# ai-dynamo/dynamo

Hardware: AMD Instinct MI355X
Metric: output tok/s (node), Llama-3-70B serving, ISL8192/OSL1024, conc 16/GPU (higher is better)
Workload: dtype bf16; 1 GPU; model=llama-3-70b, global_batch=16, seq_len=8192, osl=1024, parallelism=agg1, kv_cache_dtype=auto

## Files before the change

dynamo_amd/csrc/activation.hip:

```cpp
#include "common.h"
#include <torch/extension.h>
#include <ATen/hip/HIPContext.h>

namespace {

constexpr int kBlock = 256;

__global__ void silu_mul_kernel(short* __restrict__ out,
                                const short* __restrict__ gu,
                                int64_t T, int64_t I) {
  const int64_t nvec = T * (I / 8);
  for (int64_t v = (int64_t)blockIdx.x * kBlock + threadIdx.x; v < nvec;
       v += (int64_t)gridDim.x * kBlock) {
    const int64_t t = v / (I / 8);
    const int64_t i0 = (v % (I / 8)) * 8;
    short8 g = *reinterpret_cast<const short8*>(gu + t * 2 * I + i0);
    short8 u = *reinterpret_cast<const short8*>(gu + t * 2 * I + I + i0);
    short8 o;
#pragma unroll
    for (int i = 0; i < 8; i++) {
      float gf = bf16_to_f32(g[i]);
      float uf = bf16_to_f32(u[i]);
      float s = gf / (1.f + __expf(-gf));
      o[i] = f32_to_bf16(s * uf);
    }
    *reinterpret_cast<short8*>(out + t * I + i0) = o;
  }
}

__global__ void gelu_kernel(short* __restrict__ out, const short* __restrict__ in,
                            int64_t n) {
  const int64_t nvec = n / 8;
  for (int64_t v = (int64_t)blockIdx.x * kBlock + threadIdx.x; v < nvec;
       v += (int64_t)gridDim.x * kBlock) {
    short8 x = *reinterpret_cast<const short8*>(in + v * 8);
    short8 o;
#pragma unroll
    for (int i = 0; i < 8; i++) {
      float xf = bf16_to_f32(x[i]);
      float c = 0.7978845608028654f * (xf + 0.044715f * xf * xf * xf);
      o[i] = f32_to_bf16(0.5f * xf * (1.f + tanhf(c)));
    }
    *reinterpret_cast<short8*>(out + v * 8) = o;
  }
}

}

void silu_mul(torch::Tensor out, torch::Tensor gate_up) {
  TORCH_CHECK(out.is_cuda() && out.dtype() == torch::kBFloat16);
  TORCH_CHECK(gate_up.is_contiguous() && out.is_contiguous());
  const int64_t I = out.size(-1);
  const int64_t T = out.numel() / I;
  TORCH_CHECK(gate_up.size(-1) == 2 * I && I % 8 == 0);
  if (T == 0) return;
  const int64_t nvec = T * (I / 8);
  const int grid = (int)std::min<int64_t>((nvec + kBlock - 1) / kBlock, 2048);
  auto stream = at::cuda::getCurrentHIPStream();
// ... 17 lines not shown
```

dynamo_amd/csrc/bindings.cpp:

```cpp
#include <torch/extension.h>
#include <pybind11/pybind11.h>

namespace py = pybind11;

void rmsnorm(torch::Tensor out, torch::Tensor input, torch::Tensor weight,
             double eps, bool allow_fast);
void fused_add_rmsnorm(torch::Tensor input, torch::Tensor residual,
                       torch::Tensor weight, double eps, bool allow_fast);
void rope_append_qkv(torch::Tensor q_out, torch::Tensor kcache,
                     torch::Tensor vcache, torch::Tensor qkv,
                     c10::optional<torch::Tensor> bias,
                     torch::Tensor positions, torch::Tensor slot_mapping,
                     torch::Tensor cos_sin_cache, bool v_transposed,
                     bool allow_fast);
void rope_inplace(torch::Tensor q, torch::Tensor k, torch::Tensor positions,
                  torch::Tensor cos_sin_cache, int64_t num_q_heads,
                  int64_t num_k_heads, int64_t head_dim);
void silu_mul(torch::Tensor out, torch::Tensor gate_up);
void gelu(torch::Tensor out, torch::Tensor input);
void kv_cache_append(torch::Tensor kcache, torch::Tensor vcache, torch::Tensor k,
                     torch::Tensor v, torch::Tensor slot_mapping,
                     bool v_transposed);
void gather_pages(torch::Tensor staging, torch::Tensor cache, torch::Tensor page_ids);
void scatter_pages(torch::Tensor staging, torch::Tensor cache, torch::Tensor page_ids);
void copy_pages(torch::Tensor dst_cache, torch::Tensor src_cache, torch::Tensor pairs);
int64_t paged_decode_num_chunks(int64_t max_ctx);
int64_t decode_chunk_tokens_py(int64_t max_ctx);
void paged_attention_decode(torch::Tensor out, torch::Tensor q, torch::Tensor kcache,
                            torch::Tensor vcache, torch::Tensor page_table,
                            torch::Tensor ctx_lens, torch::Tensor partial,
                            torch::Tensor ml, double scale,
                            int64_t chunk_tokens, bool v_transposed,
                            int64_t nt_policy);
void attention_prefill_paged(torch::Tensor out, torch::Tensor q,
                             torch::Tensor kcache, torch::Tensor vcache,
                             torch::Tensor page_table, torch::Tensor tile_seq,
                             torch::Tensor tile_q0, torch::Tensor seq_q_start,
                             torch::Tensor seq_q_len, torch::Tensor seq_ctx_len,
                             double scale, bool v_transposed);
void greedy_sample(torch::Tensor out, torch::Tensor logits, bool allow_fast);
void topkp_sample(torch::Tensor out, torch::Tensor logits,
                  torch::Tensor inv_temp, torch::Tensor top_k,
                  torch::Tensor top_p, int64_t seed,
                  c10::optional<torch::Tensor> row_seeds);
void gumbel_sample(torch::Tensor out, torch::Tensor logits, torch::Tensor inv_temp,
                   int64_t seed, c10::optional<torch::Tensor> row_seeds,
                   bool allow_fast);
void penalty_fold(torch::Tensor counts, torch::Tensor slot,
                  torch::Tensor token, torch::Tensor is_prompt);
void logits_process(torch::Tensor logits, c10::optional<torch::Tensor> counts,
                    torch::Tensor slot, torch::Tensor params,
                    c10::optional<torch::Tensor> bias_off,
                    c10::optional<torch::Tensor> bias_ids,
                    c10::optional<torch::Tensor> bias_vals, bool allow_fast);
void skinny_gemm(torch::Tensor y, torch::Tensor x, torch::Tensor w,
                 int64_t wpb, int64_t u, int64_t nt, bool nontemporal,
                 bool coalesced);
std::map<std::string, std::vector<std::tuple<int, int, int>>>
skinny_gemm_configs();
void fp8_skinny_gemm(torch::Tensor y, torch::Tensor x, torch::Tensor wq,
                     torch::Tensor scale, int64_t wpb, int64_t u, int64_t nt,
                     bool nontemporal);
void fp8_dequant(torch::Tensor out, torch::Tensor wq, torch::Tensor scale);
void mxfp4_skinny_gemm(torch::Tensor y, torch::Tensor x, torch::Tensor q,
                       torch::Tensor scale, int64_t wpb, int64_t u,
                       int64_t nt, bool nontemporal);
int64_t mxfp4_gemm_max_m();
void mxfp4_dequant(torch::Tensor out, torch::Tensor q, torch::Tensor scale);
void lora_shrink(torch::Tensor t, torch::Tensor x, torch::Tensor A_bank,
                 torch::Tensor slots, torch::Tensor ranks);
void lora_expand_add(torch::Tensor y, torch::Tensor t, torch::Tensor B_bank,
                     torch::Tensor slots, torch::Tensor ranks,
                     torch::Tensor scales);
void moe_grouped_gemm(torch::Tensor y, torch::Tensor x, torch::Tensor w,
                      torch::Tensor tiles);
void moe_grouped_gemm_seg(torch::Tensor y, torch::Tensor x, torch::Tensor w,
                          torch::Tensor seg_start, int64_t max_tokens);
void topk_gating(torch::Tensor topw, torch::Tensor topi, torch::Tensor logits);
torch::Tensor ipc_alloc(int64_t nbytes, int64_t device);
py::bytes ipc_export(torch::Tensor t);
torch::Tensor ipc_open(py::bytes handle_bytes, int64_t nbytes, int64_t device);
void enable_peer_access(int64_t device, int64_t peer);
torch::Tensor mfma_probe(torch::Tensor A, torch::Tensor B);
torch::Tensor tr16_probe();
torch::Tensor vstage_probe();
torch::Tensor pv_probe(int64_t hot);

PYBIND11_MODULE(TORCH_EXTENSION_NAME, m) {
  m.doc() = "dynamo_amd native MI355X (gfx950) kernels";
  m.def("rmsnorm", &rmsnorm, py::arg("out"), py::arg("input"),
        py::arg("weight"), py::arg("eps"), py::arg("allow_fast") = true);
  m.def("fused_add_rmsnorm", &fused_add_rmsnorm, py::arg("input"),
        py::arg("residual"), py::arg("weight"), py::arg("eps"),
        py::arg("allow_fast") = true);
  m.def("rope_inplace", &rope_inplace);
  m.def("rope_append_qkv", &rope_append_qkv,
        py::arg("q_out"), py::arg("kcache"), py::arg("vcache"),
        py::arg("qkv"), py::arg("bias"), py::arg("positions"),
        py::arg("slot_mapping"), py::arg("cos_sin"),
// ... 4 lines not shown
        py::arg("vcache"), py::arg("k"), py::arg("v"),
        py::arg("slot_mapping"), py::arg("v_transposed") = false);
  m.def("gather_pages", &gather_pages);
  m.def("scatter_pages", &scatter_pages);
  m.def("copy_pages", &copy_pages);
  m.def("paged_decode_num_chunks", &paged_decode_num_chunks);
  m.def("decode_chunk_tokens", &decode_chunk_tokens_py);
  m.def("paged_attention_decode", &paged_attention_decode,
        py::arg("out"), py::arg("q"), py::arg("kcache"), py::arg("vcache"),
        py::arg("page_table"), py::arg("ctx_lens"), py::arg("partial"),
        py::arg("ml"), py::arg("scale"), py::arg("chunk_tokens"),
        py::arg("v_transposed") = false, py::arg("nt_policy") = -1);
  m.def("attention_prefill_paged", &attention_prefill_paged,
        py::arg("out"), py::arg("q"), py::arg("kcache"), py::arg("vcache"),
        py::arg("page_table"), py::arg("tile_seq"), py::arg("tile_q0"),
        py::arg("seq_q_start"), py::arg("seq_q_len"), py::arg("seq_ctx_len"),
        py::arg("scale"), py::arg("v_transposed") = false);
  m.def("greedy_sample", &greedy_sample, py::arg("out"), py::arg("logits"),
        py::arg("allow_fast") = true);
  m.def("gumbel_sample", &gumbel_sample, py::arg("out"), py::arg("logits"),
        py::arg("inv_temp"), py::arg("seed"),
        py::arg("row_seeds") = py::none(), py::arg("allow_fast") = true);
  m.def("topkp_sample", &topkp_sample, py::arg("out"), py::arg("logits"),
        py::arg("inv_temp"), py::arg("top_k"), py::arg("top_p"),
        py::arg("seed"), py::arg("row_seeds") = py::none());
  m.def("penalty_fold", &penalty_fold, py::arg("counts"), py::arg("slot"),
        py::arg("token"), py::arg("is_prompt"));
  m.def("logits_process", &logits_process, py::arg("logits"),
        py::arg("counts"), py::arg("slot"), py::arg("params"),
        py::arg("bias_off") = py::none(), py::arg("bias_ids") = py::none(),
        py::arg("bias_vals") = py::none(), py::arg("allow_fast") = true);
  m.def("skinny_gemm", &skinny_gemm, py::arg("y"), py::arg("x"), py::arg("w"),
        py::arg("wpb") = 4, py::arg("u") = 4, py::arg("nt") = 2,
        py::arg("nontemporal") = false, py::arg("coalesced") = false);
  m.def("fp8_skinny_gemm", &fp8_skinny_gemm, py::arg("y"), py::arg("x"),
        py::arg("wq"), py::arg("scale"), py::arg("wpb") = 1, py::arg("u") = 1,
        py::arg("nt") = 2, py::arg("nontemporal") = true);
  m.def("fp8_dequant", &fp8_dequant, py::arg("out"), py::arg("wq"),
        py::arg("scale"));
  m.def("mxfp4_skinny_gemm", &mxfp4_skinny_gemm, py::arg("y"), py::arg("x"),
        py::arg("q"), py::arg("scale"), py::arg("wpb") = 1, py::arg("u") = 1,
        py::arg("nt") = 2, py::arg("nontemporal") = true);
  m.def("mxfp4_gemm_max_m", &mxfp4_gemm_max_m);
  m.def("mxfp4_dequant", &mxfp4_dequant, py::arg("out"), py::arg("q"),
        py::arg("scale"));
  m.def("skinny_gemm_configs", &skinny_gemm_configs);
  m.def("lora_shrink", &lora_shrink, py::arg("t"), py::arg("x"),
        py::arg("A_bank"), py::arg("slots"), py::arg("ranks"));
  m.def("lora_expand_add", &lora_expand_add, py::arg("y"), py::arg("t"),
        py::arg("B_bank"), py::arg("slots"), py::arg("ranks"),
        py::arg("scales"));
  m.def("moe_grouped_gemm", &moe_grouped_gemm);
  m.def("moe_grouped_gemm_seg", &moe_grouped_gemm_seg);
  m.def("topk_gating", &topk_gating);
  m.def("ipc_alloc", &ipc_alloc);
  m.def("ipc_export", &ipc_export);
  m.def("ipc_open", &ipc_open);
  m.def("enable_peer_access", &enable_peer_access);
  m.def("mfma_probe", &mfma_probe);
  m.def("tr16_probe", &tr16_probe);
  m.def("vstage_probe", &vstage_probe);
  m.def("pv_probe", &pv_probe);
}
```

dynamo_amd/csrc/common.h:

```cpp
#pragma once

#include <hip/hip_runtime.h>
#include <hip/hip_bf16.h>
#include <hip/hip_fp16.h>
#include <stdint.h>

#define WAVE_SIZE 64

#define DEVINL __device__ __forceinline__

typedef __attribute__((ext_vector_type(8))) short short8;
typedef __attribute__((ext_vector_type(4))) short short4v;
typedef __attribute__((ext_vector_type(4))) float float4v;
typedef __attribute__((ext_vector_type(2))) float float2v;

typedef __attribute__((ext_vector_type(8))) short bf16x8;
typedef __attribute__((ext_vector_type(4))) float f32x4;
typedef __attribute__((ext_vector_type(16))) float f32x16;

DEVINL float bf16_to_f32(short u) {
  union { float f; uint32_t i; } v;
  v.i = ((uint32_t)(uint16_t)u) << 16;
  return v.f;
}

DEVINL short f32_to_bf16(float f) {
  union { float f; uint32_t i; } v;
  v.f = f;
  uint32_t lsb = (v.i >> 16) & 1;
  uint32_t rounded = v.i + 0x7fff + lsb;
  return (short)(rounded >> 16);
}

DEVINL float wave_reduce_sum(float x) {
#pragma unroll
  for (int off = 32; off > 0; off >>= 1) x += __shfl_xor(x, off, WAVE_SIZE);
  return x;
}

DEVINL float wave_reduce_max(float x) {
#pragma unroll
  for (int off = 32; off > 0; off >>= 1) x = fmaxf(x, __shfl_xor(x, off, WAVE_SIZE));
  return x;
}

template <int WIDTH>
DEVINL float group_reduce_sum(float x) {
#pragma unroll
  for (int off = WIDTH / 2; off > 0; off >>= 1) x += __shfl_xor(x, off, WAVE_SIZE);
  return x;
}

DEVINL float block_reduce_sum(float x, float* lds_scratch) {
  const int lane = threadIdx.x & (WAVE_SIZE - 1);
  const int wid = threadIdx.x / WAVE_SIZE;
  const int nwaves = blockDim.x / WAVE_SIZE;
  x = wave_reduce_sum(x);
  if (lane == 0) lds_scratch[wid] = x;
  __syncthreads();
  float total = 0.f;
  if (threadIdx.x < (unsigned)nwaves) total = lds_scratch[threadIdx.x];
  if (wid == 0) {
#pragma unroll
    for (int off = 8; off > 0; off >>= 1) total += __shfl_xor(total, off, WAVE_SIZE);
// ... 75 lines not shown
```

dynamo_amd/csrc/skinny_gemm.hip:

```cpp
#include "skinny_gemm_impl.h"
#include <torch/extension.h>
#include <ATen/hip/HIPContext.h>

namespace {

struct GemmArgs {
  const short* x;
  const void* w;
  const void* scale;
  short* y;
  int M, N, K;
  int64_t wpb, u, nt;
  bool nontemporal;
};

GemmArgs check_args(const char* name, int64_t max_m, int64_t min_k,
                    int64_t k_per_step, const torch::Tensor& y,
                    const torch::Tensor& x, const torch::Tensor& w,
                    const torch::Tensor* scale, int64_t wpb, int64_t u,
                    int64_t nt, bool nontemporal, int64_t w_pack = 1,
                    bool block_scaled = false) {
  TORCH_CHECK(x.is_cuda() && w.is_cuda() && y.is_cuda() &&
                  (!scale || scale->is_cuda()),
              name, ": tensors must be on the GPU");
  TORCH_CHECK(x.dtype() == torch::kBFloat16 && y.dtype() == torch::kBFloat16,
              name, ": x and y must be bf16");
  TORCH_CHECK(x.dim() == 2 && w.dim() == 2 && y.dim() == 2 &&
                  (!scale || scale->dim() == (block_scaled ? 2 : 1)),
              name, ": x [M,K], w [N,K], scale [N], y [M,N]");
  TORCH_CHECK(x.is_contiguous() && w.is_contiguous() && y.is_contiguous() &&
                  (!scale || scale->is_contiguous()),
              name, ": tensors must be contiguous");
  const int64_t M = x.size(0), K = x.size(1), N = w.size(0);
  TORCH_CHECK(w.size(1) * w_pack == K && y.size(0) == M && y.size(1) == N &&
                  (!scale || scale->size(0) == N) &&
                  (!block_scaled || scale->size(1) * 32 == K),
              name, ": shape mismatch");
  TORCH_CHECK(M >= 1 && M <= max_m, name, ": needs 1 <= M <= ", max_m,
              ", got ", M);
  TORCH_CHECK(N >= 16 && N % 16 == 0, name, ": needs N % 16 == 0, got ", N);
  TORCH_CHECK(N < (1 << 27), name, ": N too large");
  TORCH_CHECK(wpb > 0 && u > 0 && nt > 0, name, ": bad configuration");
  const int64_t kstep = wpb * k_per_step * u;
  TORCH_CHECK(K >= min_k && K < (1 << 30) && K % kstep == 0, name,
              ": needs K >= ", min_k, " and K % ", kstep, " == 0, got ", K);
  TORCH_CHECK((uintptr_t)x.data_ptr() % 16 == 0 &&
                  (uintptr_t)w.data_ptr() % 16 == 0,
              name, ": x and w must be 16 B aligned");
  TORCH_CHECK(!block_scaled || (uintptr_t)scale->data_ptr() % 8 == 0, name,
              ": scale must be 8 B aligned");
  return {(const short*)x.data_ptr(), w.data_ptr(),
          scale ? scale->data_ptr() : nullptr,
          (short*)y.data_ptr(), (int)M, (int)N, (int)K, wpb, u, nt,
          nontemporal};
}

template <class F, int WPB, int U, int NT, int MT>
void launch(const GemmArgs& a) {
  if constexpr (MT > 1) {
    if (a.M <= (MT - 1) * 16) return launch<F, WPB, U, NT, MT - 1>(a);
  }
  const int grid = (a.N + NT * 16 - 1) / (NT * 16);
  auto stream = at::cuda::getCurrentHIPStream();
  auto w = (const typename F::welem*)a.w;
  auto scale = (const typename F::scale_t*)a.scale;
  if (a.nontemporal)
    skinny::skinny_gemm_kernel<F, WPB, U, NT, MT, 1>
        <<<grid, WPB * 64, 0, stream>>>(a.x, w, scale, a.y, a.M, a.N, a.K);
  else
    skinny::skinny_gemm_kernel<F, WPB, U, NT, MT, 0>
        <<<grid, WPB * 64, 0, stream>>>(a.x, w, scale, a.y, a.M, a.N, a.K);
}

typedef std::vector<std::tuple<int, int, int>> ConfigList;

#define GEMM_CASE(WPB, U, NT)                                                \
  if (a.wpb == WPB && a.u == U && a.nt == NT)                                \
    return launch<Format, WPB, U, NT, kMaxMt>(a);
#define GEMM_ENTRY(WPB, U, NT) {WPB, U, NT},
#define GEMM_DISPATCH(NAME, F, MAX_MT, TABLE)                                \
  void NAME(const char* name, const GemmArgs& a) {                           \
    using Format = F;                                                        \
    constexpr int kMaxMt = MAX_MT;                                           \
    TABLE(GEMM_CASE)                                                         \
    TORCH_CHECK(false, name, ": no kernel for (WPB, U, NT) = (", a.wpb,      \
                ", ", a.u, ", ", a.nt, ")");                                 \
  }                                                                          \
  ConfigList NAME##_configs() { return {TABLE(GEMM_ENTRY)}; }
GEMM_DISPATCH(launch_plain, skinny::Bf16Plain, 1, SKINNY_GEMM_CONFIGS)
GEMM_DISPATCH(launch_coal, skinny::Bf16Coal, 1, SKINNY_GEMM_COAL_CONFIGS)
GEMM_DISPATCH(launch_fp8, skinny::Fp8Coal, 4, FP8_GEMM_CONFIGS)
GEMM_DISPATCH(launch_mxfp4, skinny::Mxfp4Coal, MXFP4_GEMM_MAX_MT,
              MXFP4_GEMM_CONFIGS)
#undef GEMM_DISPATCH
#undef GEMM_ENTRY
#undef GEMM_CASE

}

void skinny_gemm(torch::Tensor y, torch::Tensor x, torch::Tensor w,
                 int64_t wpb, int64_t u, int64_t nt, bool nontemporal,
                 bool coalesced) {
  const char* name = "skinny_gemm";
  TORCH_CHECK(w.dtype() == torch::kBFloat16, name, ": w must be bf16");
  const GemmArgs a = check_args(
      name, 16, 2048,
      coalesced ? skinny::Bf16Coal::KSTEP : skinny::Bf16Plain::KSTEP, y, x, w,
      nullptr, wpb, u, nt, nontemporal);
  if (coalesced) launch_coal(name, a);
  else launch_plain(name, a);
  HIP_CHECK_KERNEL();
}

void fp8_skinny_gemm(torch::Tensor y, torch::Tensor x, torch::Tensor wq,
                     torch::Tensor scale, int64_t wpb, int64_t u, int64_t nt,
                     bool nontemporal) {
  const char* name = "fp8_skinny_gemm";
  TORCH_CHECK(wq.dtype() == at::kFloat8_e4m3fn, name,
              ": wq must be float8_e4m3fn");
  TORCH_CHECK(scale.dtype() == torch::kFloat32, name, ": scale must be fp32");
  launch_fp8(name, check_args(name, 64, 128, skinny::Fp8Coal::KSTEP, y, x, wq,
                              &scale, wpb, u, nt, nontemporal));
  HIP_CHECK_KERNEL();
}

void mxfp4_skinny_gemm(torch::Tensor y, torch::Tensor x, torch::Tensor q,
                       torch::Tensor scale, int64_t wpb, int64_t u,
                       int64_t nt, bool nontemporal) {
  const char* name = "mxfp4_skinny_gemm";
  TORCH_CHECK(q.dtype() == torch::kUInt8 && scale.dtype() == torch::kUInt8,
              name, ": q and scale must be uint8");
  launch_mxfp4(name, check_args(name, 16 * MXFP4_GEMM_MAX_MT, 256,
                                skinny::Mxfp4Coal::KSTEP, y, x, q, &scale,
                                wpb, u, nt, nontemporal,
                                skinny::Mxfp4Coal::WPACK, true));
  HIP_CHECK_KERNEL();
}

std::map<std::string, ConfigList> skinny_gemm_configs() {
  return {{"bf16_plain", launch_plain_configs()},
          {"bf16_coalesced", launch_coal_configs()},
          {"fp8", launch_fp8_configs()},
          {"mxfp4", launch_mxfp4_configs()}};
}

int64_t mxfp4_gemm_max_m() { return 16 * MXFP4_GEMM_MAX_MT; }

void fp8_dequant(torch::Tensor out, torch::Tensor wq, torch::Tensor scale) {
  TORCH_CHECK(out.is_cuda() && wq.is_cuda() && scale.is_cuda(),
              "fp8_dequant: tensors must be on the GPU");
  TORCH_CHECK(out.dtype() == torch::kBFloat16 &&
                  wq.dtype() == at::kFloat8_e4m3fn &&
                  scale.dtype() == torch::kFloat32,
              "fp8_dequant: out bf16, wq float8_e4m3fn, scale fp32");
  TORCH_CHECK(out.dim() == 2 && wq.dim() == 2 && scale.dim() == 1,
              "fp8_dequant: out [N,K], wq [N,K], scale [N]");
  TORCH_CHECK(out.is_contiguous() && wq.is_contiguous() &&
                  scale.is_contiguous(),
              "fp8_dequant: tensors must be contiguous");
  const int64_t N = wq.size(0), K = wq.size(1);
  TORCH_CHECK(out.size(0) == N && out.size(1) == K && scale.size(0) == N,
              "fp8_dequant: shape mismatch");
  TORCH_CHECK(N >= 1 && K >= 16 && K % 16 == 0,
              "fp8_dequant: needs K % 16 == 0, got ", K);
  TORCH_CHECK((uintptr_t)out.data_ptr() % 16 == 0 &&
                  (uintptr_t)wq.data_ptr() % 16 == 0,
              "fp8_dequant: out and wq must be 16 B aligned");
  const int64_t threads = N * (K / 16);
  const int64_t blocks = (threads + 255) / 256;
  TORCH_CHECK(blocks < (1ll << 31), "fp8_dequant: matrix too large");
  auto stream = at::cuda::getCurrentHIPStream();
  skinny::fp8_dequant_kernel<<<(unsigned)blocks, 256, 0, stream>>>(
      (short*)out.data_ptr(), (const unsigned char*)wq.data_ptr(),
      (const float*)scale.data_ptr(), (long long)N, (long long)K);
  HIP_CHECK_KERNEL();
}
// ... 31 lines not shown
```

dynamo_amd/csrc/skinny_gemm_impl.h:

```cpp
#pragma once

#include "common.h"

namespace skinny {

typedef __attribute__((ext_vector_type(4))) int int4v;

template <int NTL>
DEVINL int4v ldw(const void* p) {
  if constexpr (NTL)
    return __builtin_nontemporal_load(reinterpret_cast<const int4v*>(p));
  else
    return *reinterpret_cast<const int4v*>(p);
}

#if !defined(__HIP_DEVICE_COMPILE__)
DEVINL bf16x8 e4m3x8_to_bf16x8(int, int) { return bf16x8{}; }
#else
DEVINL bf16x8 e4m3x8_to_bf16x8(int w0, int w1) {
  const float2v f[4] = {__builtin_amdgcn_cvt_pk_f32_fp8(w0, false),
                        __builtin_amdgcn_cvt_pk_f32_fp8(w0, true),
                        __builtin_amdgcn_cvt_pk_f32_fp8(w1, false),
                        __builtin_amdgcn_cvt_pk_f32_fp8(w1, true)};
  unsigned int out[4];
#pragma unroll
  for (int i = 0; i < 4; i++) {
    const float lo = f[i].x, hi = f[i].y;
    out[i] = __builtin_amdgcn_perm(__float_as_uint(hi), __float_as_uint(lo),
                                   0x07060302u);
  }
  return *reinterpret_cast<bf16x8*>(out);
}
#endif

typedef __attribute__((ext_vector_type(2))) __bf16 bf16x2;
// ... 66 lines not shown
  typedef CoalSel Sel;
  static constexpr int KSTEP = 128, LOADS = 2, FRAGS = 4, WPACK = 1;
  static constexpr bool SCALED = true, BLOCK_SCALED = false;
  static DEVINL int w_row(int lane, int h) { return coal_w_row(lane, h); }
  static DEVINL int w_k(int lane) { return (lane & 7) * 16; }
  static DEVINL int x_k(int lane) { return (lane >> 4) * 16; }
  static constexpr int x_step(int s) { return 64 * (s >> 1) + 8 * (s & 1); }
  static DEVINL Sel sel(int lane) { return coal_sel(lane); }
  static DEVINL bf16x8 b_frag(int s, const int4v (&r)[2], Sel l, Aux) {
    return e4m3x8_to_bf16x8(coal_take(l, s >> 1, r, 2 * (s & 1)),
                            coal_take(l, s >> 1, r, 2 * (s & 1) + 1));
  }
};

typedef __attribute__((ext_vector_type(2))) unsigned int uint2v;
struct Mxfp4Coal {
  typedef unsigned char welem;
  typedef unsigned char scale_t;
  typedef uint2v Aux;
  struct Sel { CoalSel c; int shift; };
  static constexpr int KSTEP = 256, LOADS = 2, FRAGS = 8, WPACK = 2;
  static constexpr bool SCALED = false, BLOCK_SCALED = true;
  static DEVINL int w_row(int lane, int h) { return coal_w_row(lane, h); }
  static DEVINL int w_k(int lane) { return (lane & 7) * 16; }
  static DEVINL int x_k(int lane) { return (lane >> 4) * 32; }
  static constexpr int x_step(int s) { return 128 * (s >> 2) + 8 * (s & 3); }
  static DEVINL Sel sel(int lane) { return {coal_sel(lane), (lane >> 4) * 8}; }
  static DEVINL bf16x8 b_frag(int s, const int4v (&r)[2], Sel l, Aux a) {
    return e2m1x8_to_bf16x8(coal_take(l.c, s >> 2, r, s & 3),
                            (a[s >> 2] >> l.shift) & 0xffu);
  }
};

template <class F, int WPB, int U, int NT, int MT, int NTL>
__global__ __launch_bounds__(WPB * 64) void skinny_gemm_kernel(
    const short* __restrict__ x,
    const typename F::welem* __restrict__ w,
    const typename F::scale_t* __restrict__ scale,
    short* __restrict__ y,
    int M, int N, int K) {
  const int lane = threadIdx.x & 63;
  const int wid = threadIdx.x >> 6;
  const int lr = lane & 15;
  const int lg = lane >> 4;
  const int n0 = (blockIdx.x * NT) * 16;
  if (n0 >= N) return;

  const int kw = K / WPB;
  const int k0 = wid * kw;
  const int steps = kw / F::KSTEP;

  const short* xp[MT];
#pragma unroll
  for (int m = 0; m < MT; m++) {
    const int row = m * 16 + lr;
    xp[m] = x + (size_t)(row < M ? row : 0) * K + k0 + F::x_k(lane);
  }
  const typename F::welem* wp[NT][F::LOADS];
#pragma unroll
  for (int t = 0; t < NT; t++)
#pragma unroll
    for (int h = 0; h < F::LOADS; h++) {
      const int col = n0 + t * 16 + F::w_row(lane, h);
      wp[t][h] = w + (size_t)(col < N ? col : N - 1) * (K / F::WPACK) +
                 k0 / F::WPACK + F::w_k(lane);
    }
  const typename F::scale_t* sp[NT];
  if constexpr (F::BLOCK_SCALED) {
#pragma unroll
    for (int t = 0; t < NT; t++) {
      const int col = n0 + t * 16 + lr;
      sp[t] = scale + ((size_t)(col < N ? col : N - 1) * K + k0) / 32;
    }
  }

  const typename F::Sel sel = F::sel(lane);

  f32x4 acc[NT][MT];
#pragma unroll
  for (int t = 0; t < NT; t++)
#pragma unroll
    for (int m = 0; m < MT; m++) acc[t][m] = f32x4{0.f, 0.f, 0.f, 0.f};

  bf16x8 abuf[U][MT][F::FRAGS];
  int4v rbuf[NT][U][F::LOADS];
  typename F::Aux auxbuf[NT][U];
  auto load_x = [&](bf16x8 (&a)[MT][F::FRAGS], int d) {
#pragma unroll
    for (int m = 0; m < MT; m++)
#pragma unroll
      for (int s = 0; s < F::FRAGS; s++)
        a[m][s] = *reinterpret_cast<const bf16x8*>(xp[m] + d * F::KSTEP +
                                                   F::x_step(s));
  };
  auto load_w = [&](int4v (&r)[F::LOADS], typename F::Aux& ax, int t, int d) {
#pragma unroll
    for (int h = 0; h < F::LOADS; h++)
      r[h] = ldw<NTL>(wp[t][h] + d * (F::KSTEP / F::WPACK));
    if constexpr (F::BLOCK_SCALED)
      ax = *reinterpret_cast<const typename F::Aux*>(sp[t] +
                                                     d * (F::KSTEP / 32));
  };
  auto consume = [&](const bf16x8 (&a)[MT][F::FRAGS],
                     const int4v (&r)[F::LOADS], typename F::Aux ax,
                     f32x4 (&c)[MT]) {
// ... 32 lines not shown
        consume(a, r, ax, acc[t]);
      }
    }
  }
#pragma unroll
  for (int u = 0; u < U; u++)
#pragma unroll
    for (int t = 0; t < NT; t++)
      consume(abuf[u], rbuf[t][u], auxbuf[t][u], acc[t]);

  __shared__ f32x4 red[WPB > 1 ? (WPB - 1) * NT * 64 : 1];
  if (WPB > 1) {
#pragma unroll
    for (int m = 0; m < MT; m++) {
      if (m > 0) __syncthreads();
      if (wid > 0) {
#pragma unroll
        for (int t = 0; t < NT; t++)
          red[((wid - 1) * NT + t) * 64 + lane] = acc[t][m];
      }
      __syncthreads();
      if (wid == 0) {
#pragma unroll
        for (int t = 0; t < NT; t++)
#pragma unroll
          for (int r = 0; r < WPB - 1; r++) {
            f32x4 o = red[(r * NT + t) * 64 + lane];
            acc[t][m].x += o.x; acc[t][m].y += o.y;
            acc[t][m].z += o.z; acc[t][m].w += o.w;
          }
      }
    }
    if (wid > 0) return;
  }
#pragma unroll
  for (int t = 0; t < NT; t++) {
    const int col = n0 + t * 16 + lr;
    if (col >= N) continue;
    float sc = 1.f;
    if constexpr (F::SCALED) sc = scale[col];
#pragma unroll
    for (int m = 0; m < MT; m++)
#pragma unroll
      for (int i = 0; i < 4; i++) {
        const int row = m * 16 + lg * 4 + i;
        if (row < M) {
          float v = acc[t][m][i];
          if constexpr (F::SCALED) v *= sc;
          y[(size_t)row * N + col] = f32_to_bf16(v);
        }
      }
  }
}

__global__ __launch_bounds__(256) void fp8_dequant_kernel(
    short* __restrict__ out, const unsigned char* __restrict__ wq,
    const float* __restrict__ scale, long long N, long long K) {
  const long long chunks = K / 16;
  const long long i = (long long)blockIdx.x * blockDim.x + threadIdx.x;
  if (i >= N * chunks) return;
  const long long row = i / chunks;
  const float sc = scale[row];
  const int4v v = *reinterpret_cast<const int4v*>(wq + i * 16);
  short8 o[2];
#if defined(__HIP_DEVICE_COMPILE__)
#pragma unroll
// ... 14 lines not shown
  op[1] = o[1];
}

__global__ __launch_bounds__(256) void mxfp4_dequant_kernel(
    short* __restrict__ out, const unsigned char* __restrict__ q,
    const unsigned char* __restrict__ scale, long long blocks) {
  const long long i = (long long)blockIdx.x * blockDim.x + threadIdx.x;
  if (i >= blocks) return;
  const unsigned int e = scale[i];
  const int4v v = *reinterpret_cast<const int4v*>(q + i * 16);
  bf16x8* op = reinterpret_cast<bf16x8*>(out + i * 32);
#pragma unroll
  for (int j = 0; j < 4; j++) op[j] = e2m1x8_to_bf16x8((unsigned int)v[j], e);
}

#define SKINNY_GEMM_CONFIGS(X)                               \
  X(4, 4, 2) X(4, 4, 4) X(4, 2, 4) X(2, 4, 4) X(2, 8, 4)                    \
  X(1, 8, 4) X(1, 4, 8) X(2, 4, 8) X(4, 8, 2) X(2, 2, 8) X(4, 8, 4)          \
  X(8, 4, 2) X(16, 4, 2) X(16, 2, 2) X(8, 4, 1) X(16, 4, 1) X(8, 2, 4)

#define SKINNY_GEMM_COAL_CONFIGS(X)                           \
  X(8, 1, 2) X(8, 1, 4) X(8, 2, 2) X(4, 2, 2) X(8, 2, 4) X(2, 2, 8)          \
  X(1, 4, 2) X(1, 2, 4) X(1, 4, 4) X(1, 8, 2) X(1, 2, 2) X(1, 1, 8) X(1, 2, 8)

#define FP8_GEMM_CONFIGS(X)                                                 \
  X(1, 1, 1) X(1, 1, 2) X(1, 2, 2) X(2, 1, 4) X(2, 2, 2)                     \
  X(4, 1, 2) X(4, 2, 2) X(4, 1, 4) X(8, 1, 2) X(8, 2, 2)

#define MXFP4_GEMM_CONFIGS(X)                                               \
  X(1, 1, 1) X(1, 1, 2) X(1, 2, 2) X(2, 1, 2) X(2, 1, 4) X(4, 1, 2)          \
  X(4, 1, 4) X(4, 1, 8) X(8, 1, 2) X(8, 1, 4) X(2, 1, 8)
#define MXFP4_GEMM_MAX_MT 2

}
```

dynamo_amd/envs.py:

```python
from __future__ import annotations

import os

ENV_VARS = {
    "DYN_DISCOVERY_BACKEND": "discovery backend spec: memory | file:/path",
    "DYN_NAMESPACE": "default namespace for components",
    "DYN_LOG": "log level (INFO, DEBUG, ...)",
    "DYN_LOGGING_JSONL": "1 = structured JSONL logs",
    "DYN_REQUEST_TRACE_FILE": "JSONL request-trace sink path",
    "DYN_HTTP_PORT": "frontend HTTP port",
    "DYN_ROUTER_MODE": "kv | round_robin | random | least_loaded | p2c",
    "DYN_ROUTER_TEMPERATURE": "softmax temperature for kv routing",
    "DYN_KV_BLOCK_SIZE": "KV page size in tokens",
    "DYN_KV_GPU_MEM_FRACTION": "fraction of free HBM for the KV pool",
    "DYN_HOST_CACHE_PAGES": "KVBM G2 pinned-host tier size (pages)",
    "DYN_TUNABLEOP": "0 disables the pre-tuned hipBLASLt table",
    "DYN_WORKER_TYPE": "aggregated | prefill | decode",
    "DYN_BYPASS_TOKEN_THRESHOLD":
        "conditional disagg: net-new prefill tokens below this bypass the "
        "prefill pool (reference conditional_disagg.rs:15; default 2048)",
    "DYNAMO_DECODE_CHUNK": "decode attention context-chunk tokens override",
    "DYNAMO_DECODE_MFMA": "0 = force the VALU decode path (token-major only)",
    "DYNAMO_DECODE_SWAPPED": "0 = A-operand MFMA decode (token-major only)",
    "DYNAMO_DECODE_NT":
        "1 = non-temporal K/V loads in the d-major (VT4) decode attention "
        "kernel (bit-identical outputs; recorded-negative, slower)",
    "DYNAMO_SKINNY_GEMM":
        "0 = every decode weight GEMM on hipBLASLt (default: the in-tree "
        "skinny-M kernel on the shapes in ops.SKINNY_GEMM_SHAPES)",
    "DYNAMO_MAX_LORAS":
        "default of the worker's --max-loras: adapter-bank slots for "
        "per-request LoRA (default 0 = engine-level activation only)",
    "DYNAMO_MAX_LORA_RANK":
        "default of the worker's --max-lora-rank: the largest (fused block "
        "form) adapter rank a bank slot holds, a multiple of 8 (default 64)",
    "DYNAMO_WEIGHT_DTYPE":
        "what EngineConfig.weight_dtype=\"auto\" resolves to: bf16 (default; "
        "the compute dtype, unquantised) | fp8 (e4m3 projection weights, "
        "W8A16) | mxfp4 (OCP microscaling FP4 projection weights: e2m1 codes "
        "with one e8m0 scale per 32 k, W4A16)",
    "DYNAMO_MOE_BMM": "0 = grouped-kernel MoE decode instead of padded bmm",
    "DYNAMO_MOE_MFMA": "0 = VALU grouped MoE GEMM",
    "DYNAMO_MOE_GRAPHS": "0 = exclude MoE layers from hipGraph capture",
    "DYNAMO_ROCTX": "1 = roctx range annotations for rocprofv3 traces",
}


def get(name: str, default=None, cast=str):
    v = os.environ.get(name)
    if v is None:
        return default
    try:
        if cast is bool:
            return v not in ("0", "false", "False", "")
        return cast(v)
    except (TypeError, ValueError):
        return default


def discovery(default="memory"):
    return get("DYN_DISCOVERY_BACKEND", default)

# ... 4 lines not shown
```

dynamo_amd/models/layers.py:

```python
from __future__ import annotations

from dataclasses import dataclass, field
from typing import List, Optional

import torch
import torch.nn.functional as F

from dynamo_amd import ops


@dataclass
class AttnMetadata:
    slot_mapping: torch.Tensor
    positions: torch.Tensor
    num_decode: int = 0
    decode_page_table: Optional[torch.Tensor] = None
    decode_ctx_lens: Optional[torch.Tensor] = None
    decode_scratch: Optional["ops.DecodeScratch"] = None
    num_prefill_tokens: int = 0
    prefill_page_table: Optional[torch.Tensor] = None
    seq_q_start: Optional[torch.Tensor] = None
    seq_q_len: Optional[torch.Tensor] = None
    seq_ctx_len: Optional[torch.Tensor] = None
    prefill_tiles: Optional[tuple] = None
# ... 167 lines not shown
                qh[nd:].contiguous(), kcache, vcache, meta.prefill_page_table,
                meta.seq_q_start, meta.seq_q_len, meta.seq_ctx_len, self.scale,
                meta.prefill_tiles, v_transposed=meta.v_transposed)
        out = out.view(T, self.hq * self.hd)
        o = linear_lora(out, self.wo, self.lora, "o")
        if meta.lora_slots is not None:
            lora_bank_delta_(o, out, self.lora_bank["o"], meta)
        return self.tp.all_reduce(o)


class SwiGLUMLP(torch.nn.Module):
    def __init__(self, cfg, tp: TPContext, device, dtype):
        super().__init__()
        self.tp = tp
        D = cfg.hidden_size
        I = cfg.intermediate_size // tp.size
        self.I = I
        self.w_gate_up, needs = _alloc((2 * I, D), device, dtype)
        if needs:
            with torch.no_grad():
                for sec in range(2):
                    full = torch.empty(cfg.intermediate_size, D, device=device,
                                       dtype=dtype).normal_(0.0, 0.02)
                    self.w_gate_up[sec * I:(sec + 1) * I].copy_(
                        full[tp.rank * I:(tp.rank + 1) * I]
                        if tp.size > 1 else full)
        self.w_down = init_sharded((D, cfg.intermediate_size), device, dtype,
                                   tp, 1)
        self.lora = None
        self.lora_bank = None

    def forward(self, x, meta: Optional[AttnMetadata] = None):
        batched = meta is not None and meta.lora_slots is not None
        gu = linear_lora(x, self.w_gate_up, self.lora, "gate_up")
        if batched:
            lora_bank_delta_(gu, x, self.lora_bank["gate_up"], meta)
        act = ops.silu_mul(gu)
        down = linear_lora(act, self.w_down, self.lora, "down")
        if batched:
            lora_bank_delta_(down, act, self.lora_bank["down"], meta)
        return self.tp.all_reduce(down)
```

dynamo_amd/ops/__init__.py:

```python
from __future__ import annotations

import torch

from . import fp8_weights, mxfp4_weights, torch_ref
from .fp8_weights import (Fp8Weight, quantize_fp8_rowwise,
                          quantize_model_fp8)
from .mxfp4_weights import (Mxfp4Weight, quantize_mxfp4,
                            quantize_model_mxfp4)
from .torch_ref import make_cos_sin_cache

_hip_mod = None
_hip_err: Exception | None = None


def hip():
    global _hip_mod, _hip_err
    if _hip_mod is None:
        try:
            from dynamo_amd import _hip as m
            _hip_mod = m
        except Exception as e:
            _hip_err = e
            raise RuntimeError(
                "dynamo_amd._hip native extension is not available on a GPU "
# ... 57 lines not shown
FP8_GEMM_SHAPES: dict = {
    (10240, 8192): ((4, 1, 2), (4, 1, 4)),
    (8192, 8192): ((8, 1, 2), (4, 1, 2)),
    (57344, 8192): ((4, 1, 4), (2, 1, 4)),
    (8192, 28672): ((4, 2, 2), (4, 1, 2)),
}
FP8_GEMM_MAX_M = 64


def _quant_gemm_config(M, N, K, kstep, max_m, shapes, split_k, default):
    if not (1 <= M <= max_m and K >= kstep and K % kstep == 0
            and N >= 16 and N % 16 == 0):
        return None
    entry = shapes.get((N, K))
    cfg = entry[0 if M <= 16 else 1] if entry else split_k
    if K % (cfg[0] * kstep * cfg[1]):
        cfg = default
    return cfg


def _quant_linear_path(x, w, dequant_k, gemm_config):
    N, K = w.shape
    if not x.is_cuda:
        return "torch", None
    if x.dtype != torch.bfloat16 or K % dequant_k or x.shape[-1] != K:
        return "torch", None
    if x.dim() == 2 and x.is_contiguous() and x.data_ptr() % 16 == 0:
        cfg = gemm_config(x.shape[0], N, K)
        if cfg is not None:
            return "kernel", cfg
    return "dequant", None


def _linear_quant(x, w, path, cfg, gemm: str, dequant: str):
    if path == "kernel":
        y = torch.empty(x.shape[0], w.shape[0], dtype=x.dtype, device=x.device)
        getattr(hip(), gemm)(y, x, w.q, w.scale, *cfg, True)
        return y
    if path == "dequant":
        w_eff = fp8_weights.scratch_view(w)
        getattr(hip(), dequant)(w_eff, w.q, w.scale)
        return torch.nn.functional.linear(x, w_eff)
    return torch.nn.functional.linear(x, w.effective(x.dtype))


def fp8_gemm_config(M: int, N: int, K: int):
    return _quant_gemm_config(M, N, K, 128, FP8_GEMM_MAX_M, FP8_GEMM_SHAPES,
                              FP8_GEMM_SPLIT_K, FP8_GEMM_DEFAULT)


def fp8_linear_path(x: torch.Tensor, w: Fp8Weight):
    return _quant_linear_path(x, w, 16, fp8_gemm_config)


def _linear_fp8(x: torch.Tensor, w: Fp8Weight) -> torch.Tensor:
    return _linear_quant(x, w, *fp8_linear_path(x, w), "fp8_skinny_gemm",
                         "fp8_dequant")


MXFP4_GEMM_CONFIGS: tuple = (
    (1, 1, 1), (1, 1, 2), (1, 2, 2), (2, 1, 2), (2, 1, 4), (4, 1, 2),
    (4, 1, 4), (4, 1, 8), (8, 1, 2), (8, 1, 4), (2, 1, 8),
)
MXFP4_GEMM_DEFAULT: tuple = (1, 1, 2)
MXFP4_GEMM_SPLIT_K: tuple = (4, 1, 2)
MXFP4_GEMM_SHAPES: dict = {
    (10240, 8192): ((4, 1, 4), (8, 1, 4)),
    (8192, 8192): ((4, 1, 2), (4, 1, 2)),
    (57344, 8192): ((2, 1, 8), (2, 1, 8)),
    (8192, 28672): ((4, 1, 2), (4, 1, 2)),
}
MXFP4_GEMM_MAX_M = 32


def mxfp4_gemm_config(M: int, N: int, K: int):
    return _quant_gemm_config(M, N, K, 256, MXFP4_GEMM_MAX_M,
                              MXFP4_GEMM_SHAPES, MXFP4_GEMM_SPLIT_K,
                              MXFP4_GEMM_DEFAULT)


def mxfp4_linear_path(x: torch.Tensor, w: Mxfp4Weight):
    if w.q.data_ptr() % 16 or w.scale.data_ptr() % 8:
        return _quant_linear_path(x, w, 32, lambda M, N, K: None)
    return _quant_linear_path(x, w, 32, mxfp4_gemm_config)


def _linear_mxfp4(x: torch.Tensor, w: Mxfp4Weight) -> torch.Tensor:
    return _linear_quant(x, w, *mxfp4_linear_path(x, w), "mxfp4_skinny_gemm",
                         "mxfp4_dequant")


def linear(x: torch.Tensor, w) -> torch.Tensor:
    if isinstance(w, Fp8Weight):
        return _linear_fp8(x, w)
    if isinstance(w, Mxfp4Weight):
        return _linear_mxfp4(x, w)
    cfg = skinny_gemm_config(x, w)
    if cfg is None:
        return torch.nn.functional.linear(x, w)
    y = torch.empty(x.shape[0], w.shape[0], dtype=x.dtype, device=x.device)
    hip().skinny_gemm(y, x, w, *cfg)
    return y


def rmsnorm(x: torch.Tensor, weight: torch.Tensor, eps: float,
            allow_fast: bool = True) -> torch.Tensor:
    if x.is_cuda:
        out = torch.empty_like(x)
        hip().rmsnorm(out, x.contiguous(), weight, eps, allow_fast)
        return out
    return torch_ref.rmsnorm(x, weight, eps)


def fused_add_rmsnorm(x, residual, weight, eps, allow_fast=True):
    if x.is_cuda:
        hip().fused_add_rmsnorm(x, residual, weight, eps, allow_fast)
        return x
    return torch_ref.fused_add_rmsnorm(x, residual, weight, eps)


def rope_inplace(q, k, positions, cos_sin, num_q_heads, num_k_heads, head_dim):
    if q.is_cuda:
        hip().rope_inplace(q, k, positions, cos_sin, num_q_heads, num_k_heads,
                           head_dim)
        return q, k
    return torch_ref.rope(q, k, positions, cos_sin, num_q_heads, num_k_heads,
                          head_dim)


def silu_mul(gate_up: torch.Tensor) -> torch.Tensor:
    if gate_up.is_cuda:
        d = gate_up.shape[-1] // 2
        out = torch.empty(gate_up.shape[:-1] + (d,), dtype=gate_up.dtype,
                          device=gate_up.device)
# ... 276 lines not shown
```

Measured before the change: 456.7 tok/s.

## Fuse SwiGLU activation into the skinny GEMM epilogue for gate/up projection

Adds a GLU template mode to the skinny GEMM kernel in which each block computes paired gate and up tiles and applies silu(gate)*up in the epilogue, writing the half-width activation directly. The MLP forward uses this fused path when no LoRA is active and the GEMM config supports it, which removes the separate silu_mul launch and the write and re-read of the full gate_up intermediate. In exchange each block now covers half as many output columns per NT, and the fused path is only available for the coalesced bf16, fp8 and mxfp4 formats.

```diff
diff --git a/dynamo_amd/csrc/activation.hip b/dynamo_amd/csrc/activation.hip
--- a/dynamo_amd/csrc/activation.hip
+++ b/dynamo_amd/csrc/activation.hip
@@ -18,12 +18,7 @@
     short8 u = *reinterpret_cast<const short8*>(gu + t * 2 * I + I + i0);
     short8 o;
 #pragma unroll
-    for (int i = 0; i < 8; i++) {
-      float gf = bf16_to_f32(g[i]);
-      float uf = bf16_to_f32(u[i]);
-      float s = gf / (1.f + __expf(-gf));
-      o[i] = f32_to_bf16(s * uf);
-    }
+    for (int i = 0; i < 8; i++) o[i] = silu_mul_bf16(g[i], u[i]);
     *reinterpret_cast<short8*>(out + t * I + i0) = o;
   }
 }
diff --git a/dynamo_amd/csrc/bindings.cpp b/dynamo_amd/csrc/bindings.cpp
--- a/dynamo_amd/csrc/bindings.cpp
+++ b/dynamo_amd/csrc/bindings.cpp
@@ -55,16 +55,18 @@
                     c10::optional<torch::Tensor> bias_vals, bool allow_fast);
 void skinny_gemm(torch::Tensor y, torch::Tensor x, torch::Tensor w,
                  int64_t wpb, int64_t u, int64_t nt, bool nontemporal,
-                 bool coalesced);
+                 bool coalesced, bool glu);
 std::map<std::string, std::vector<std::tuple<int, int, int>>>
 skinny_gemm_configs();
+std::map<std::string, std::vector<std::tuple<int, int, int>>>
+skinny_gemm_glu_configs();
 void fp8_skinny_gemm(torch::Tensor y, torch::Tensor x, torch::Tensor wq,
                      torch::Tensor scale, int64_t wpb, int64_t u, int64_t nt,
-                     bool nontemporal);
+                     bool nontemporal, bool glu);
 void fp8_dequant(torch::Tensor out, torch::Tensor wq, torch::Tensor scale);
 void mxfp4_skinny_gemm(torch::Tensor y, torch::Tensor x, torch::Tensor q,
                        torch::Tensor scale, int64_t wpb, int64_t u,
-                       int64_t nt, bool nontemporal);
+                       int64_t nt, bool nontemporal, bool glu);
 int64_t mxfp4_gemm_max_m();
 void mxfp4_dequant(torch::Tensor out, torch::Tensor q, torch::Tensor scale);
 void lora_shrink(torch::Tensor t, torch::Tensor x, torch::Tensor A_bank,
@@ -135,19 +137,23 @@
         py::arg("bias_vals") = py::none(), py::arg("allow_fast") = true);
   m.def("skinny_gemm", &skinny_gemm, py::arg("y"), py::arg("x"), py::arg("w"),
         py::arg("wpb") = 4, py::arg("u") = 4, py::arg("nt") = 2,
-        py::arg("nontemporal") = false, py::arg("coalesced") = false);
+        py::arg("nontemporal") = false, py::arg("coalesced") = false,
+        py::arg("glu") = false);
   m.def("fp8_skinny_gemm", &fp8_skinny_gemm, py::arg("y"), py::arg("x"),
         py::arg("wq"), py::arg("scale"), py::arg("wpb") = 1, py::arg("u") = 1,
-        py::arg("nt") = 2, py::arg("nontemporal") = true);
+        py::arg("nt") = 2, py::arg("nontemporal") = true,
+        py::arg("glu") = false);
   m.def("fp8_dequant", &fp8_dequant, py::arg("out"), py::arg("wq"),
         py::arg("scale"));
   m.def("mxfp4_skinny_gemm", &mxfp4_skinny_gemm, py::arg("y"), py::arg("x"),
         py::arg("q"), py::arg("scale"), py::arg("wpb") = 1, py::arg("u") = 1,
-        py::arg("nt") = 2, py::arg("nontemporal") = true);
+        py::arg("nt") = 2, py::arg("nontemporal") = true,
+        py::arg("glu") = false);
   m.def("mxfp4_gemm_max_m", &mxfp4_gemm_max_m);
   m.def("mxfp4_dequant", &mxfp4_dequant, py::arg("out"), py::arg("q"),
         py::arg("scale"));
   m.def("skinny_gemm_configs", &skinny_gemm_configs);
+  m.def("skinny_gemm_glu_configs", &skinny_gemm_glu_configs);
   m.def("lora_shrink", &lora_shrink, py::arg("t"), py::arg("x"),
         py::arg("A_bank"), py::arg("slots"), py::arg("ranks"));
   m.def("lora_expand_add", &lora_expand_add, py::arg("y"), py::arg("t"),
diff --git a/dynamo_amd/csrc/common.h b/dynamo_amd/csrc/common.h
--- a/dynamo_amd/csrc/common.h
+++ b/dynamo_amd/csrc/common.h
@@ -30,6 +30,13 @@
   uint32_t lsb = (v.i >> 16) & 1;
   uint32_t rounded = v.i + 0x7fff + lsb;
   return (short)(rounded >> 16);
+}
+
+DEVINL short silu_mul_bf16(short gate, short up) {
+  float gf = bf16_to_f32(gate);
+  float uf = bf16_to_f32(up);
+  float s = gf / (1.f + __expf(-gf));
+  return f32_to_bf16(s * uf);
 }
 
 DEVINL float wave_reduce_sum(float x) {
diff --git a/dynamo_amd/csrc/skinny_gemm.hip b/dynamo_amd/csrc/skinny_gemm.hip
--- a/dynamo_amd/csrc/skinny_gemm.hip
+++ b/dynamo_amd/csrc/skinny_gemm.hip
@@ -12,14 +12,15 @@
   int M, N, K;
   int64_t wpb, u, nt;
   bool nontemporal;
+  bool glu;
 };
 
 GemmArgs check_args(const char* name, int64_t max_m, int64_t min_k,
                     int64_t k_per_step, const torch::Tensor& y,
                     const torch::Tensor& x, const torch::Tensor& w,
                     const torch::Tensor* scale, int64_t wpb, int64_t u,
-                    int64_t nt, bool nontemporal, int64_t w_pack = 1,
-                    bool block_scaled = false) {
+                    int64_t nt, bool nontemporal, bool glu,
+                    int64_t w_pack = 1, bool block_scaled = false) {
   TORCH_CHECK(x.is_cuda() && w.is_cuda() && y.is_cuda() &&
                   (!scale || scale->is_cuda()),
               name, ": tensors must be on the GPU");
@@ -32,7 +33,8 @@
                   (!scale || scale->is_contiguous()),
               name, ": tensors must be contiguous");
   const int64_t M = x.size(0), K = x.size(1), N = w.size(0);
-  TORCH_CHECK(w.size(1) * w_pack == K && y.size(0) == M && y.size(1) == N &&
+  TORCH_CHECK(w.size(1) * w_pack == K && y.size(0) == M &&
+                  y.size(1) == (glu ? N / 2 : N) &&
                   (!scale || scale->size(0) == N) &&
                   (!block_scaled || scale->size(1) * 32 == K),
               name, ": shape mismatch");
@@ -40,6 +42,9 @@
               ", got ", M);
   TORCH_CHECK(N >= 16 && N % 16 == 0, name, ": needs N % 16 == 0, got ", N);
   TORCH_CHECK(N < (1 << 27), name, ": N too large");
+  TORCH_CHECK(!glu || (N % 32 == 0 && nt % 2 == 0), name,
+              ": the fused SwiGLU form needs N % 32 == 0 and an even NT, got "
+              "N = ", N, ", NT = ", nt);
   TORCH_CHECK(wpb > 0 && u > 0 && nt > 0, name, ": bad configuration");
   const int64_t kstep = wpb * k_per_step * u;
   TORCH_CHECK(K >= min_k && K < (1 << 30) && K % kstep == 0, name,
@@ -52,32 +57,43 @@
   return {(const short*)x.data_ptr(), w.data_ptr(),
           scale ? scale->data_ptr() : nullptr,
           (short*)y.data_ptr(), (int)M, (int)N, (int)K, wpb, u, nt,
-          nontemporal};
-}
-
-template <class F, int WPB, int U, int NT, int MT>
+          nontemporal, glu};
+}
+
+template <class F, int WPB, int U, int NT, int MT, int GLU>
 void launch(const GemmArgs& a) {
   if constexpr (MT > 1) {
-    if (a.M <= (MT - 1) * 16) return launch<F, WPB, U, NT, MT - 1>(a);
+    if (a.M <= (MT - 1) * 16) return launch<F, WPB, U, NT, MT - 1, GLU>(a);
   }
   const int grid = (a.N + NT * 16 - 1) / (NT * 16);
   auto stream = at::cuda::getCurrentHIPStream();
   auto w = (const typename F::welem*)a.w;
   auto scale = (const typename F::scale_t*)a.scale;
   if (a.nontemporal)
-    skinny::skinny_gemm_kernel<F, WPB, U, NT, MT, 1>
+    skinny::skinny_gemm_kernel<F, WPB, U, NT, MT, 1, GLU>
         <<<grid, WPB * 64, 0, stream>>>(a.x, w, scale, a.y, a.M, a.N, a.K);
   else
-    skinny::skinny_gemm_kernel<F, WPB, U, NT, MT, 0>
+    skinny::skinny_gemm_kernel<F, WPB, U, NT, MT, 0, GLU>
         <<<grid, WPB * 64, 0, stream>>>(a.x, w, scale, a.y, a.M, a.N, a.K);
+}
+
+template <class F, int WPB, int U, int NT, int MT>
+void launch_form(const char* name, const GemmArgs& a) {
+  if (!a.glu) return launch<F, WPB, U, NT, MT, 0>(a);
+  if constexpr (skinny::glu_capable<F>(WPB, U, NT))
+    return launch<F, WPB, U, NT, MT, 1>(a);
+  TORCH_CHECK(false, name, ": no fused SwiGLU kernel for (WPB, U, NT) = (",
+              WPB, ", ", U, ", ", NT, ") of this format");
 }
 
 typedef std::vector<std::tuple<int, int, int>> ConfigList;
 
 #define GEMM_CASE(WPB, U, NT)                                                \
   if (a.wpb == WPB && a.u == U && a.nt == NT)                                \
-    return launch<Format, WPB, U, NT, kMaxMt>(a);
+    return launch_form<Format, WPB, U, NT, kMaxMt>(name, a);
 #define GEMM_ENTRY(WPB, U, NT) {WPB, U, NT},
+#define GEMM_GLU_ENTRY(WPB, U, NT)                                           \
+  if (skinny::glu_capable<Format>(WPB, U, NT)) l.push_back({WPB, U, NT});
 #define GEMM_DISPATCH(NAME, F, MAX_MT, TABLE)                                \
   void NAME(const char* name, const GemmArgs& a) {                           \
     using Format = F;                                                        \
@@ -86,13 +102,20 @@
     TORCH_CHECK(false, name, ": no kernel for (WPB, U, NT) = (", a.wpb,      \
                 ", ", a.u, ", ", a.nt, ")");                                 \
   }                                                                          \
-  ConfigList NAME##_configs() { return {TABLE(GEMM_ENTRY)}; }
+  ConfigList NAME##_configs() { return {TABLE(GEMM_ENTRY)}; }              \
+  ConfigList NAME##_glu_configs() {                                          \
+    using Format = F;                                                        \
+    ConfigList l;                                                            \
+    TABLE(GEMM_GLU_ENTRY)                                                    \
+    return l;                                                                \
+  }
 GEMM_DISPATCH(launch_plain, skinny::Bf16Plain, 1, SKINNY_GEMM_CONFIGS)
 GEMM_DISPATCH(launch_coal, skinny::Bf16Coal, 1, SKINNY_GEMM_COAL_CONFIGS)
 GEMM_DISPATCH(launch_fp8, skinny::Fp8Coal, 4, FP8_GEMM_CONFIGS)
 GEMM_DISPATCH(launch_mxfp4, skinny::Mxfp4Coal, MXFP4_GEMM_MAX_MT,
               MXFP4_GEMM_CONFIGS)
 #undef GEMM_DISPATCH
+#undef GEMM_GLU_ENTRY
 #undef GEMM_ENTRY
 #undef GEMM_CASE
 
@@ -100,13 +123,13 @@
 
 void skinny_gemm(torch::Tensor y, torch::Tensor x, torch::Tensor w,
                  int64_t wpb, int64_t u, int64_t nt, bool nontemporal,
-                 bool coalesced) {
+                 bool coalesced, bool glu) {
   const char* name = "skinny_gemm";
   TORCH_CHECK(w.dtype() == torch::kBFloat16, name, ": w must be bf16");
   const GemmArgs a = check_args(
       name, 16, 2048,
       coalesced ? skinny::Bf16Coal::KSTEP : skinny::Bf16Plain::KSTEP, y, x, w,
-      nullptr, wpb, u, nt, nontemporal);
+      nullptr, wpb, u, nt, nontemporal, glu);
   if (coalesced) launch_coal(name, a);
   else launch_plain(name, a);
   HIP_CHECK_KERNEL();
@@ -114,25 +137,25 @@
 
 void fp8_skinny_gemm(torch::Tensor y, torch::Tensor x, torch::Tensor wq,
                      torch::Tensor scale, int64_t wpb, int64_t u, int64_t nt,
-                     bool nontemporal) {
+                     bool nontemporal, bool glu) {
   const char* name = "fp8_skinny_gemm";
   TORCH_CHECK(wq.dtype() == at::kFloat8_e4m3fn, name,
               ": wq must be float8_e4m3fn");
   TORCH_CHECK(scale.dtype() == torch::kFloat32, name, ": scale must be fp32");
   launch_fp8(name, check_args(name, 64, 128, skinny::Fp8Coal::KSTEP, y, x, wq,
-                              &scale, wpb, u, nt, nontemporal));
+                              &scale, wpb, u, nt, nontemporal, glu));
   HIP_CHECK_KERNEL();
 }
 
 void mxfp4_skinny_gemm(torch::Tensor y, torch::Tensor x, torch::Tensor q,
                        torch::Tensor scale, int64_t wpb, int64_t u,
-                       int64_t nt, bool nontemporal) {
+                       int64_t nt, bool nontemporal, bool glu) {
   const char* name = "mxfp4_skinny_gemm";
   TORCH_CHECK(q.dtype() == torch::kUInt8 && scale.dtype() == torch::kUInt8,
               name, ": q and scale must be uint8");
   launch_mxfp4(name, check_args(name, 16 * MXFP4_GEMM_MAX_MT, 256,
                                 skinny::Mxfp4Coal::KSTEP, y, x, q, &scale,
-                                wpb, u, nt, nontemporal,
+                                wpb, u, nt, nontemporal, glu,
                                 skinny::Mxfp4Coal::WPACK, true));
   HIP_CHECK_KERNEL();
 }
@@ -142,6 +165,13 @@
           {"bf16_coalesced", launch_coal_configs()},
           {"fp8", launch_fp8_configs()},
           {"mxfp4", launch_mxfp4_configs()}};
+}
+
+std::map<std::string, ConfigList> skinny_gemm_glu_configs() {
+  return {{"bf16_plain", launch_plain_glu_configs()},
+          {"bf16_coalesced", launch_coal_glu_configs()},
+          {"fp8", launch_fp8_glu_configs()},
+          {"mxfp4", launch_mxfp4_glu_configs()}};
 }
 
 int64_t mxfp4_gemm_max_m() { return 16 * MXFP4_GEMM_MAX_MT; }
diff --git a/dynamo_amd/csrc/skinny_gemm_impl.h b/dynamo_amd/csrc/skinny_gemm_impl.h
--- a/dynamo_amd/csrc/skinny_gemm_impl.h
+++ b/dynamo_amd/csrc/skinny_gemm_impl.h
@@ -1,6 +1,7 @@
 #pragma once
 
 #include "common.h"
+#include <type_traits>
 
 namespace skinny {
 
@@ -133,19 +134,22 @@
   }
 };
 
-template <class F, int WPB, int U, int NT, int MT, int NTL>
+template <class F, int WPB, int U, int NT, int MT, int NTL, int GLU = 0>
 __global__ __launch_bounds__(WPB * 64) void skinny_gemm_kernel(
     const short* __restrict__ x,
     const typename F::welem* __restrict__ w,
     const typename F::scale_t* __restrict__ scale,
     short* __restrict__ y,
     int M, int N, int K) {
+  static_assert(!GLU || NT % 2 == 0, "GLU pairs gate and up tiles");
   const int lane = threadIdx.x & 63;
   const int wid = threadIdx.x >> 6;
   const int lr = lane & 15;
   const int lg = lane >> 4;
-  const int n0 = (blockIdx.x * NT) * 16;
-  if (n0 >= N) return;
+  constexpr int NTO = GLU ? NT / 2 : NT;
+  const int NO = GLU ? N / 2 : N;
+  const int n0 = (blockIdx.x * NTO) * 16;
+  if (n0 >= NO) return;
 
   const int kw = K / WPB;
   const int k0 = wid * kw;
@@ -162,16 +166,20 @@
   for (int t = 0; t < NT; t++)
 #pragma unroll
     for (int h = 0; h < F::LOADS; h++) {
-      const int col = n0 + t * 16 + F::w_row(lane, h);
-      wp[t][h] = w + (size_t)(col < N ? col : N - 1) * (K / F::WPACK) +
+      int col = n0 + (t % NTO) * 16 + F::w_row(lane, h);
+      col = col < NO ? col : NO - 1;
+      if (GLU && t >= NTO) col += NO;
+      wp[t][h] = w + (size_t)col * (K / F::WPACK) +
                  k0 / F::WPACK + F::w_k(lane);
     }
   const typename F::scale_t* sp[NT];
   if constexpr (F::BLOCK_SCALED) {
 #pragma unroll
     for (int t = 0; t < NT; t++) {
-      const int col = n0 + t * 16 + lr;
-      sp[t] = scale + ((size_t)(col < N ? col : N - 1) * K + k0) / 32;
+      int col = n0 + (t % NTO) * 16 + lr;
+      col = col < NO ? col : NO - 1;
+      if (GLU && t >= NTO) col += NO;
+      sp[t] = scale + ((size_t)col * K + k0) / 32;
     }
   }
 
@@ -270,6 +278,28 @@
       }
     }
     if (wid > 0) return;
+  }
+  if constexpr (GLU) {
+#pragma unroll
+    for (int t = 0; t < NTO; t++) {
+      const int col = n0 + t * 16 + lr;
+      if (col >= NO) continue;
+      float sg = 1.f, su = 1.f;
+      if constexpr (F::SCALED) { sg = scale[col]; su = scale[col + NO]; }
+#pragma unroll
+      for (int m = 0; m < MT; m++)
+#pragma unroll
+        for (int i = 0; i < 4; i++) {
+          const int row = m * 16 + lg * 4 + i;
+          if (row < M) {
+            float g = acc[t][m][i], u = acc[t + NTO][m][i];
+            if constexpr (F::SCALED) { g *= sg; u *= su; }
+            y[(size_t)row * NO + col] =
+                silu_mul_bf16(f32_to_bf16(g), f32_to_bf16(u));
+          }
+        }
+    }
+    return;
   }
 #pragma unroll
   for (int t = 0; t < NT; t++) {
@@ -350,4 +380,10 @@
   X(4, 1, 4) X(4, 1, 8) X(8, 1, 2) X(8, 1, 4) X(2, 1, 8)
 #define MXFP4_GEMM_MAX_MT 2
 
-}
+template <class F>
+constexpr bool glu_capable(int wpb, int u, int nt) {
+  if (std::is_same<F, Bf16Plain>::value || nt % 2) return false;
+  return !(std::is_same<F, Bf16Coal>::value && wpb == 8 && u == 1 && nt == 4);
+}
+
+}
diff --git a/dynamo_amd/envs.py b/dynamo_amd/envs.py
--- a/dynamo_amd/envs.py
+++ b/dynamo_amd/envs.py
@@ -28,6 +28,10 @@
     "DYNAMO_SKINNY_GEMM":
         "0 = every decode weight GEMM on hipBLASLt (default: the in-tree "
         "skinny-M kernel on the shapes in ops.SKINNY_GEMM_SHAPES)",
+    "DYNAMO_FUSED_GLU":
+        "0 = gate/up GEMM and silu_mul as two kernels (default: the in-tree "
+        "GEMM applies SwiGLU in its epilogue where ops.fused_glu_config "
+        "allows; equal bits either way)",
     "DYNAMO_MAX_LORAS":
         "default of the worker's --max-loras: adapter-bank slots for "
         "per-request LoRA (default 0 = engine-level activation only)",
diff --git a/dynamo_amd/models/layers.py b/dynamo_amd/models/layers.py
--- a/dynamo_amd/models/layers.py
+++ b/dynamo_amd/models/layers.py
@@ -223,10 +223,13 @@
 
     def forward(self, x, meta: Optional[AttnMetadata] = None):
         batched = meta is not None and meta.lora_slots is not None
-        gu = linear_lora(x, self.w_gate_up, self.lora, "gate_up")
-        if batched:
-            lora_bank_delta_(gu, x, self.lora_bank["gate_up"], meta)
-        act = ops.silu_mul(gu)
+        if not batched and not (self.lora and "gate_up" in self.lora):
+            act = ops.linear_silu_mul(x, self.w_gate_up)
+        else:
+            gu = linear_lora(x, self.w_gate_up, self.lora, "gate_up")
+            if batched:
+                lora_bank_delta_(gu, x, self.lora_bank["gate_up"], meta)
+            act = ops.silu_mul(gu)
         down = linear_lora(act, self.w_down, self.lora, "down")
         if batched:
             lora_bank_delta_(down, act, self.lora_bank["down"], meta)
diff --git a/dynamo_amd/ops/__init__.py b/dynamo_amd/ops/__init__.py
--- a/dynamo_amd/ops/__init__.py
+++ b/dynamo_amd/ops/__init__.py
@@ -113,10 +113,11 @@
     return "dequant", None
 
 
-def _linear_quant(x, w, path, cfg, gemm: str, dequant: str):
+def _linear_quant(x, w, path, cfg, gemm: str, dequant: str, glu=False):
     if path == "kernel":
-        y = torch.empty(x.shape[0], w.shape[0], dtype=x.dtype, device=x.device)
-        getattr(hip(), gemm)(y, x, w.q, w.scale, *cfg, True)
+        y = torch.empty(x.shape[0], w.shape[0] // 2 if glu else w.shape[0],
+                        dtype=x.dtype, device=x.device)
+        getattr(hip(), gemm)(y, x, w.q, w.scale, *cfg, True, glu)
         return y
     if path == "dequant":
         w_eff = fp8_weights.scratch_view(w)
@@ -181,6 +182,62 @@
         return torch.nn.functional.linear(x, w)
     y = torch.empty(x.shape[0], w.shape[0], dtype=x.dtype, device=x.device)
     hip().skinny_gemm(y, x, w, *cfg)
+    return y
+
+
+FUSED_GLU_FORMATS: tuple = ("bf16_coalesced", "fp8", "mxfp4")
+
+_fused_glu_override: "bool | None" = None
+
+
+def set_fused_glu(on: "bool | None") -> None:
+    global _fused_glu_override
+    _fused_glu_override = on
+
+
+def fused_glu_enabled() -> bool:
+    if _fused_glu_override is not None:
+        return _fused_glu_override
+    from dynamo_amd import envs
+    return envs.get("DYNAMO_FUSED_GLU", True, bool)
+
+
+def glu_capable(fmt: str, cfg) -> bool:
+    if fmt == "bf16_plain" or cfg[2] % 2:
+        return False
+    return not (fmt == "bf16_coalesced" and tuple(cfg[:3]) == (8, 1, 4))
+
+
+def fused_glu_config(x: torch.Tensor, w):
+    if not fused_glu_enabled() or w.shape[0] % 32:
+        return None
+    if isinstance(w, Fp8Weight):
+        path, cfg = fp8_linear_path(x, w)
+        hit = ("fp8_skinny_gemm", "fp8", cfg) if path == "kernel" else None
+    elif isinstance(w, Mxfp4Weight):
+        path, cfg = mxfp4_linear_path(x, w)
+        hit = (("mxfp4_skinny_gemm", "mxfp4", cfg) if path == "kernel"
+               else None)
+    else:
+        cfg = skinny_gemm_config(x, w)
+        hit = None if cfg is None else (
+            "skinny_gemm", "bf16_coalesced" if cfg[4] else "bf16_plain", cfg)
+    if (hit is None or hit[1] not in FUSED_GLU_FORMATS
+            or not glu_capable(hit[1], hit[2])):
+        return None
+    return hit[0], hit[2]
+
+
+def linear_silu_mul(x: torch.Tensor, w_gate_up) -> torch.Tensor:
+    hit = fused_glu_config(x, w_gate_up)
+    if hit is None:
+        return silu_mul(linear(x, w_gate_up))
+    gemm, cfg = hit
+    if gemm != "skinny_gemm":
+        return _linear_quant(x, w_gate_up, "kernel", cfg, gemm, None, True)
+    y = torch.empty(x.shape[0], w_gate_up.shape[0] // 2, dtype=x.dtype,
+                    device=x.device)
+    hip().skinny_gemm(y, x, w_gate_up, *cfg, True)
     return y
 
 
```

Measured after the change: 465.4 tok/s (median of 6 runs). 1.02x the previous value.
